# Simon-Kotchou/ViT.rs

Measured on AMD Instinct MI355X. Metric: images/sec (train step) ViT-B/16 224² bf16 at 1/2/4/8 MI355X; % MFMA roofline, higher is better.
Workload: dtype bf16; 1 GPU; vit_b16 224x224 train step (fwd+bwd+SGD), batch 256/GPU, bf16; model=vit_b16, global_batch=256, seq_len=197, parallelism=dp1

## Files before the change

### vit.rs_amd/csrc/gemm.h

```cpp
#pragma once
#include "common.h"

namespace vit {

enum Epi {
    EPI_F32_STORE = 0,
    EPI_F32_ACC = 1,
    EPI_F32_ATOMIC = 2,
    EPI_BF16_STORE = 3,
    EPI_BF16_GELU = 4,
    EPI_F32_RESID = 5,
    EPI_BF16_DGELU = 6,
    EPI_F32_SLAB = 7,
    EPI_BF16_GELU_D = 8,
    EPI_BF16_MUL = 9,
};
constexpr bool epi_aux16(int e) { return e == EPI_BF16_DGELU || e == EPI_BF16_MUL; }
constexpr bool epi_bias(int e) { return e != EPI_F32_ATOMIC && e != EPI_F32_SLAB && !epi_aux16(e); }
constexpr bool epi_mx(int e) { return e == EPI_BF16_GELU || e == EPI_BF16_GELU_D || epi_aux16(e); }

struct GemmArgs {
    const void* A = nullptr;
    long long lda = 0;
    bool a_kcontig = true;
    const void* B = nullptr;
    long long ldb = 0;
    bool b_kcontig = true;
    void* C = nullptr;
    long long ldc = 0;
    void* C2 = nullptr;
    const void* aux = nullptr;
    long long ldaux = 0;
    const float* bias = nullptr;
    float* dbias = nullptr;
    float* colsum_out = nullptr;
    float* colsum_part = nullptr;
    int M = 0, N = 0, K = 0;
    int epi = EPI_F32_STORE;
    int splitk = 0;
    int fill_pct = 0;
    float* ws = nullptr;
    size_t ws_bytes = 0;
    const void* a_scale = nullptr;
    const void* b_scale = nullptr;
    uint8_t* mx_q = nullptr;
    uint8_t* mx_s = nullptr;
    uint8_t* mxc_q = nullptr;
    uint8_t* mxc_s = nullptr;
    long long mxc_ld = 0;
    long long mxc_off = 0;
};

void gemm_f32(const GemmArgs& a, hipStream_t s);
void gemm_bf16(const GemmArgs& a, hipStream_t s);
bool gemm_bf16_supported(const GemmArgs& a);
void gemm_set_variant(int v);
void gemm_set_debug(int flags);
int gemm_cu_count();
int gemm_persist_grid();
struct GemmParams;
void gemm_set_trace(unsigned long long* trace);
bool gemm_pp_shape(const GemmArgs& a);
void gemm_bf16_pp(const GemmArgs& a, const GemmParams& p, hipStream_t s);
// ... 48 lines not shown
```

### vit.rs_amd/csrc/gemm.hip

```cpp
#include "gemm_common.h"

#include <cstdlib>

#ifndef VIT_G2_ONEPHASE
#define VIT_G2_ONEPHASE 0
#endif

namespace vit {

namespace bf {
constexpr int BM = 128, BN = 128, BK = 64, NT = 256;
constexpr int SK = 72;
constexpr int SMN = 144;
constexpr int TILE = 9216;
static_assert(BM * SK == TILE && BK * SMN == TILE, "image sizes");

template <bool KC, int ROWS>
struct Stager {
    uint4 r[4];
    __device__ __forceinline__ void load(const bf16_t* __restrict__ base, long long ld, int row0,
                                         int rows_lim, int k0, int k_lim, int tid) {
#pragma unroll
        for (int c = 0; c < 4; c++) {
            const int idx = c * NT + tid;
// ... 1187 lines not shown
    if (slab) slab_reduce(a, slab, split, s);
    if (a.dbias) colsum_bf16(a.dbias, (const bf16_t*)a.A, a.K, a.M, a.lda, s);
}

void gemm_bf16(const GemmArgs& a, hipStream_t s) {
    if (a.M <= 0 || a.N <= 0) return;
    if (a.mx_q || a.mxc_q) {
        set_error("gemm_bf16: the fused MX output is an fp8-engine feature");
        return;
    }
    if (!gemm_bf16_supported(a)) {
        set_error("gemm_bf16: unsupported shape/alignment M=%d N=%d K=%d lda=%lld ldb=%lld",
                  a.M, a.N, a.K, a.lda, a.ldb);
        return;
    }
    if (gemm_variant() != 1 && a.epi == EPI_F32_ATOMIC && !a.a_kcontig && !a.b_kcontig &&
        a.K % g4::KTILE == 0 && a.M >= 256 && a.N >= 128 && a.N % 4 == 0 &&
        (a.splitk > 0 || !a.ws ||
         (size_t)choose_split_g4(cdiv(a.M, g4::BM) * cdiv(a.N, g4::BN), a.K / g4::KTILE) * a.M * a.N * sizeof(float) <=
             a.ws_bytes)) {
        gemm_bf16_g4(a, s);
        return;
    }
    const bool big = a.K % g2::KTILE == 0 && a.M >= 256 && a.N >= 256 && gemm_variant() != 1;
    if (big) {
        const int tiles = cdiv(a.M, g2::BM) * cdiv(a.N, g2::BN);
        int split = 1;
        if (a.epi == EPI_F32_ATOMIC) split = a.splitk > 0 ? a.splitk : choose_split_waves(tiles, a.K / g2::KTILE);
        int kchunk = cdiv(cdiv(a.K, split), g2::KTILE) * g2::KTILE;
        split = cdiv(a.K, kchunk);
        GemmArgs b = a;
        float* slab = nullptr;
        if (a.epi == EPI_F32_ATOMIC) {
            if (split > 1) {
                if (!(slab = slab_buffer(a, split))) return;
                b.epi = EPI_F32_SLAB;
                b.C = slab;
                b.ldc = a.N;
            } else {
                b.epi = EPI_F32_ACC;
            }
        }
        GemmParams p = make_gemm_params(b, kchunk);
        p.tiles = tiles;
        float* cs_rows = colsum_rows_begin(a);
        if ((a.colsum_out || a.colsum_part) && epi_aux16(a.epi) && !cs_rows) return;
        p.colsum_out = cs_rows;
// ... 69 lines not shown
```

### vit.rs_amd/csrc/ops.hip

```cpp
#include "ops_internal.h"
#include "ln_common.h"

namespace vit {

__global__ void residual_fwd_k(float* __restrict__ out, const float* __restrict__ a,
                               const float* __restrict__ b, long long n) {
    for (long long i = blockIdx.x * (long long)blockDim.x + threadIdx.x; i < n;
         i += (long long)gridDim.x * blockDim.x)
        out[i] = a[i] + b[i];
}
__global__ void residual_bwd_k(float* __restrict__ d1, float* __restrict__ d2,
                               const float* __restrict__ dout, long long n) {
    for (long long i = blockIdx.x * (long long)blockDim.x + threadIdx.x; i < n;
         i += (long long)gridDim.x * blockDim.x) {
        const float g = dout[i];
        d1[i] += g;
        d2[i] += g;
    }
}
__global__ void gelu_fwd_k(float* __restrict__ out, const float* __restrict__ inp, long long n) {
    for (long long i = blockIdx.x * (long long)blockDim.x + threadIdx.x; i < n;
         i += (long long)gridDim.x * blockDim.x)
        out[i] = gelu_f(inp[i]);
}
// ... 101 lines not shown
    }
}
__global__ void f2bf_k(bf16_t* __restrict__ out, const float* __restrict__ inp, long long n) {
    for (long long i = blockIdx.x * (long long)blockDim.x + threadIdx.x; i < n;
         i += (long long)gridDim.x * blockDim.x)
        out[i] = f2bf(inp[i]);
}
__global__ void bf2f_k(float* __restrict__ out, const bf16_t* __restrict__ inp, long long n) {
    for (long long i = blockIdx.x * (long long)blockDim.x + threadIdx.x; i < n;
         i += (long long)gridDim.x * blockDim.x)
        out[i] = bf2f(inp[i]);
}

int grid_for(long long n, int threads) {
    long long b = (n + threads - 1) / threads;
    return (int)(b < 1 ? 1 : (b > 8192 ? 8192 : b));
}

template <typename TO>
__global__ __launch_bounds__(256) void ln_fwd_k(TO* __restrict__ out, float* __restrict__ mean,
                                                float* __restrict__ rstd,
                                                const float* __restrict__ inp,
                                                const float* __restrict__ w,
                                                const float* __restrict__ b, long long rows, int C) {
    const int lane = threadIdx.x & 63;
    const long long row = blockIdx.x * 4LL + (threadIdx.x >> 6);
    if (row >= rows) return;
    const float* x = inp + row * C;
    float s = 0.f;
    for (int i = lane; i < C; i += 64) s += x[i];
    const float m = warp_sum(s) / (float)C;
    float v = 0.f;
    for (int i = lane; i < C; i += 64) {
        const float d = x[i] - m;
        v += d * d;
    }
    v = warp_sum(v) / (float)C;
    const float r = 1.0f / sqrtf(v + 1e-5f);
    TO* o = out + row * C;
    for (int i = lane; i < C; i += 64) {
        const float y = (r * (x[i] - m)) * w[i] + b[i];
        if constexpr (sizeof(TO) == 2)
            o[i] = f2bf(y);
        else
            o[i] = y;
    }
    if (lane == 0) {
        mean[row] = m;
        rstd[row] = r;
    }
// ... 55 lines not shown
            dval -= nrm * dnorm_norm_mean;
            dval *= rs;
            const long long o = row * C + i;
            if constexpr (ST) {
                const float t = lo8_decode(bf2f(io.hi_in[o]), io.lo_in[o]) + dval;
                const bf16_t h = f2bf(t);
                io.hi_out[o] = h;
                io.lo_out[o] = (uint8_t)lo8_encode(t, bf2f(h));
                ps[i] += t;
            } else {
                io.dinp[o] += dval;
            }
        }
    }
    lnb_flush(io, sm, C);
}

template <int NV, typename TO>
__global__ __launch_bounds__(256) void ln_fwd_vec_k(TO* __restrict__ out, float* __restrict__ mean,
                                                    float* __restrict__ rstd,
                                                    const float* __restrict__ inp,
                                                    const float* __restrict__ w,
                                                    const float* __restrict__ b, long long rows,
                                                    int C) {
    const int lane = threadIdx.x & 63;
    const long long row = blockIdx.x * 4LL + (threadIdx.x >> 6);
    if (row >= rows) return;
    const float4* x4 = reinterpret_cast<const float4*>(inp + row * C);
    float4 v[NV];
#pragma unroll
    for (int j = 0; j < NV; j++) v[j] = x4[lane + 64 * j];
    float m, r;
    ln_vec_stats<NV>(v, C, m, r);
#pragma unroll
    for (int j = 0; j < NV; j++) {
        const int k = lane + 64 * j;
        const float4 y = ln_vec_y(v[j], reinterpret_cast<const float4*>(w)[k], reinterpret_cast<const float4*>(b)[k], m, r);
        if constexpr (sizeof(TO) == 2)
            reinterpret_cast<uint2*>(out + row * C)[k] = make_uint2(pack_bf16x2(y.x, y.y), pack_bf16x2(y.z, y.w));
        else
            reinterpret_cast<float4*>(out + row * C)[k] = y;
    }
    if (lane == 0) {
        mean[row] = m;
        rstd[row] = r;
    }
}

__device__ __forceinline__ float4 ld4(const float* p, int k) { return reinterpret_cast<const float4*>(p)[k]; }
__device__ __forceinline__ float4 ld4(const bf16_t* p, int k) {
// ... 403 lines not shown
    float s = 0.f;
    for (int y = 0; y < nch; y++) s += part[y * n + i];
    dwpe[i] += s;
    tsum[i] = s;
}
__global__ void patch_small_grads_fin_k(float* __restrict__ dcls, float* __restrict__ dpb,
                                        const float* __restrict__ tsum, int T, int C) {
    const int c = blockIdx.x * blockDim.x + threadIdx.x;
    if (c >= C) return;
    float ps[8] = {0.f, 0.f, 0.f, 0.f, 0.f, 0.f, 0.f, 0.f};
    int t = 1;
    for (; t + 8 <= T; t += 8) {
#pragma unroll
        for (int j = 0; j < 8; j++) ps[j] += tsum[(long long)(t + j) * C + c];
    }
    for (int j = 0; t < T; t++, j++) ps[j] += tsum[(long long)t * C + c];
    const float s = ((ps[0] + ps[1]) + (ps[2] + ps[3])) + ((ps[4] + ps[5]) + (ps[6] + ps[7]));
    dcls[c] += tsum[c];
    dpb[c] += s;
}

template <typename TO>
static void ln_forward_any(TO* out, float* mean, float* rstd, const float* inp, const float* w,
                           const float* b, long long rows, int C, hipStream_t s) {
    if (rows <= 0) return;
    const int g = cdiv(rows, 4);
    const bool vec = C % 256 == 0 && C <= 2048 && (((uintptr_t)inp | (uintptr_t)out | (uintptr_t)w | (uintptr_t)b) & 15) == 0;
    switch (vec ? C / 256 : 0) {
        case 1: ln_fwd_vec_k<1, TO><<<g, 256, 0, s>>>(out, mean, rstd, inp, w, b, rows, C); break;
        case 2: ln_fwd_vec_k<2, TO><<<g, 256, 0, s>>>(out, mean, rstd, inp, w, b, rows, C); break;
        case 3: ln_fwd_vec_k<3, TO><<<g, 256, 0, s>>>(out, mean, rstd, inp, w, b, rows, C); break;
        case 4: ln_fwd_vec_k<4, TO><<<g, 256, 0, s>>>(out, mean, rstd, inp, w, b, rows, C); break;
        case 5: ln_fwd_vec_k<5, TO><<<g, 256, 0, s>>>(out, mean, rstd, inp, w, b, rows, C); break;
        case 6: ln_fwd_vec_k<6, TO><<<g, 256, 0, s>>>(out, mean, rstd, inp, w, b, rows, C); break;
        case 8: ln_fwd_vec_k<8, TO><<<g, 256, 0, s>>>(out, mean, rstd, inp, w, b, rows, C); break;
        default: ln_fwd_k<TO><<<g, 256, 0, s>>>(out, mean, rstd, inp, w, b, rows, C); break;
    }
    after_launch("layernorm_forward");
}
void ln_forward_f32(float* out, float* mean, float* rstd, const float* inp, const float* w,
                    const float* b, long long rows, int C, hipStream_t s) {
    ln_forward_any<float>(out, mean, rstd, inp, w, b, rows, C, s);
}
void ln_forward_bf16(bf16_t* out, float* mean, float* rstd, const float* inp, const float* w,
                     const float* b, long long rows, int C, hipStream_t s) {
    ln_forward_any<bf16_t>(out, mean, rstd, inp, w, b, rows, C, s);
}
int ln_bwd_blocks(long long rows);
template <typename TD, bool ST>
static void ln_backward_any(LnbIo io, const TD* dout, const float* inp, const float* w,
                            const float* mean, const float* rstd, long long rows, int C, hipStream_t s,
                            float* ws = nullptr) {
    if (rows <= 0) return;
    const bool reduce = io.part == nullptr;
    const int nsum = io.dsum ? 3 * C : 2 * C;
    if (reduce) {
        io.part = ws ? ws : (float*)workspace((size_t)ln_bwd_blocks(rows) * nsum * sizeof(float));
        if (!io.part) return;
    }
    const bool vec = C % 256 == 0 && C <= 2048 &&
                     (((uintptr_t)io.dinp | (uintptr_t)dout | (uintptr_t)inp | (uintptr_t)w |
                       (uintptr_t)io.hi_in | (uintptr_t)io.hi_out | (uintptr_t)io.lo_in | (uintptr_t)io.lo_out) & 15) == 0;
    const int grid = ln_bwd_blocks(rows);
    const size_t lds = 12 * (size_t)C * sizeof(float);
    if (lds > 160 * 1024) { set_error("layernorm_backward: C=%d exceeds the LDS column partials", C); return; }
    if (!vec) {
        if (lds > 64 * 1024) VIT_HIP(hipFuncSetAttribute((const void*)ln_bwd_k<TD, ST>,
                                                         hipFuncAttributeMaxDynamicSharedMemorySize, (int)lds));
        ln_bwd_k<TD, ST><<<grid, 256, lds, s>>>(io, dout, inp, w, mean, rstd, rows, C);
// ... 499 lines not shown
```

### vit.rs_amd/csrc/ops_internal.h

```cpp
#pragma once
#include "common.h"
#include "gemm.h"
#include "../../include/vit_ops.h"

namespace vit {
int grid_for(long long n, int threads);
void ln_forward_f32(float* out, float* mean, float* rstd, const float* inp, const float* w,
                    const float* b, long long rows, int C, hipStream_t s);
void ln_forward_bf16(bf16_t* out, float* mean, float* rstd, const float* inp, const float* w,
                     const float* b, long long rows, int C, hipStream_t s);
void ln_backward_f32(float* dinp, float* dw, float* db, const float* dout, const float* inp,
                     const float* w, const float* mean, const float* rstd, long long rows, int C,
                     hipStream_t s, float* ws = nullptr);
void ln_backward_bf16_stream(bf16_t* dres_out, uint8_t* lo_out, const bf16_t* dres_in, const uint8_t* lo_in,
                             float* dw, float* db, float* dres_colsum, const bf16_t* dout, const float* inp,
                             const float* w, const float* mean, const float* rstd, long long rows, int C,
                             hipStream_t s, float* part = nullptr);
int ln_bwd_blocks(long long rows);
void convert_f2bf(bf16_t* out, const float* inp, long long n, hipStream_t s);
void sgd(float* p, const float* g, long long n, float lr, hipStream_t s);
void sgd_clip(float* p, const float* g, long long n, float lr, const ClipRec* rec, hipStream_t s);
int group_grid(int ntiles);
void sgd_groups(float* p, const float* g, const GroupTab& gt, int tile_begin, int ntiles, float lr,
                const ClipRec* rec, hipStream_t s);
int sumsq_blocks(long long n);
void sumsq_partials(double* slots, const float* x, long long n, hipStream_t s);
void sumsq_finish(double* out, const double* slots, int nslots, hipStream_t s);
void clip_finish(ClipRec* rec, const double* slots, int nslots, float max_norm, hipStream_t s);
void softmax_rows(float* probs, const float* logits, long long rows, int V, hipStream_t s);
void ce_forward(float* losses, const float* probs, const int* targets, long long rows, int V,
                hipStream_t s);
void ce_backward(float* dlogits, const float* dlosses, const float* probs, const int* targets,
                 long long rows, int V, hipStream_t s);
// ... 38 lines not shown
```

### vit.rs_amd/csrc/trainer.hip

```cpp
#include <rccl/rccl.h>

#include <algorithm>
#include <cmath>
#include <cstdlib>
#include <cstring>
#include <string>
#include <vector>

#include "ops_internal.h"
#include "../../include/vit_trainer.h"
#include "../../include/vit_checkpoint.h"
#include "../../include/vit_data.h"
#include "../../include/vit_jpeg.h"

namespace vit {
bool jpeg_loader_decode_to(vit_jpeg_loader_t* l, uint8_t* out, int img, hipStream_t st, const int** labels,
                           int expect_n);
namespace {

enum TIdx {
    P_PATCH_W, P_PATCH_B, P_CLS, P_WPE, P_LN1W, P_LN1B, P_QKVW, P_QKVB, P_ATTPROJW, P_ATTPROJB,
    P_LN2W, P_LN2B, P_FCW, P_FCB, P_FCPROJW, P_FCPROJB, P_LNFW, P_LNFB, P_HEADW, P_HEADB
};

// ... 239 lines not shown
}

struct DevBuf {
    void* p = nullptr;
    size_t bytes = 0;
};

}

struct Trainer {
    vit_config_t cfg{};
    int B = 0, T = 0, NP = 0, C = 0, L = 0, NH = 0, NC = 0, KP = 0, prec = 0, device = 0;
    long long BT = 0;
    long long n_params = 0;
    long long arena_elems = 0;
    long long canon_size[20]{};
    std::vector<long long> off;
    long long chunk_off[VIT_MAX_LAYERS + 3]{};
    int n_chunks = 0;

    hipStream_t s = nullptr, s_comm = nullptr;
    hipStream_t s2 = nullptr;
    bool two_streams = true;
    enum BwdEv { EV_RESA, EV_RESB, EV_DFCH, EV_DQKV, EV_W1, EV_W2, EV_W3, EV_W4, EV_JOIN, EV_SG, EV_PRE_IN, EV_PRE, EV_COUNT };
    hipEvent_t bev[EV_COUNT]{};
    static constexpr int MAXMB = 4;
    int nmb = 1, mb_want = 2;
    int pick_nmb(int want) const {
        if (!two_streams) return 1;
        for (int k = want < MAXMB ? want : MAXMB; k >= 2; k--)
            if (B % k == 0) return k;
        return 1;
    }
    hipStream_t ms[MAXMB]{};
    hipEvent_t mev[MAXMB][EV_COUNT]{};
    hipEvent_t fork_ev = nullptr, join_ev[MAXMB]{};
    std::vector<hipEvent_t> chunk_evm;
    std::vector<hipEvent_t> chunk_ev2;
    std::vector<hipEvent_t> chunk_ev;
    hipEvent_t comm_done = nullptr;

    float* params = nullptr;
    float* grads = nullptr;
    float* gemm_ws = nullptr;
    float* attn_part = nullptr;
    size_t gemm_ws_bytes = 0;
    bf16_t* pbf = nullptr;
// ... 341 lines not shown
            } else {
                patches_bf = alloc<bf16_t>((long long)B * NP * KPP);
            }
            if (patch_pad) {
                wpatch_pad = alloc<bf16_t>((long long)C * KPP);
                dwpatch_pad = alloc<float>((long long)C * KPP);
                if (wpatch_pad) VIT_HIP(hipMemset(wpatch_pad, 0, (size_t)C * KPP * 2));
            }
            for (int l = 0; l < L; l++) {
                LayerActs& a = la[l];
                a.ln1 = alloc<bf16_t>(BT * C);
                a.ln1_mean = alloc<float>(BT);
                a.ln1_rstd = alloc<float>(BT);
                a.qkv = alloc<bf16_t>(BT * 3 * C);
                a.atty = alloc<bf16_t>(BT * C);
                a.lse = alloc<float>(BT * NH);
                a.res2 = alloc<float>(BT * C);
                a.ln2 = alloc<bf16_t>(BT * C);
                a.ln2_mean = alloc<float>(BT);
                a.ln2_rstd = alloc<float>(BT);
                a.fchd = alloc<bf16_t>(BT * 4 * C);
                a.fchg = alloc<bf16_t>(BT * 4 * C);
                a.res3 = alloc<float>(BT * C);
            }
            dln_bf = alloc<bf16_t>(BT * C);
            dres_bf = alloc<bf16_t>(BT * C);
            dres_bf2 = alloc<bf16_t>(BT * C);
            dres_lo = alloc<uint8_t>(BT * C);
            dres_lo2 = alloc<uint8_t>(BT * C);
            dfch = alloc<bf16_t>(BT * 4 * C);
            datty = alloc<bf16_t>(BT * C);
            dqkv = alloc<bf16_t>(BT * 3 * C);
            if (!patch_f32) dpatch_bf = alloc<bf16_t>((long long)B * NP * C);
            gemm_ws_bytes = (size_t)32 * 4 * C * (size_t)std::max(C, KP) * sizeof(float);
            gemm_ws = alloc<float>((long long)(gemm_ws_bytes / sizeof(float)));
            attn_part = alloc<float>((long long)attn_backward_ws_floats(B, T, C, NH) + MAXMB * 3LL * C);
            {
                const long long lnr = (long long)MAXMB * ln_bwd_blocks(BT), fcr = cdiv(BT, 96) + MAXMB;
                sg_ln2 = 0;
                sg_ln1 = sg_ln2 + lnr * 3 * C;
                sg_fcb = sg_ln1 + lnr * 3 * C;
                sg_qkv = sg_fcb + fcr * 4 * C;
                const long long n = sg_qkv + (long long)MAXMB * 3 * C;
                sg_part[0] = alloc<float>(n);
                sg_part[1] = alloc<float>(n);
            }
// ... 201 lines not shown
            aq = act_q2[mb];
            as = act_s2[mb];
        } else if (pre == PRE_NONE) {
            tbeg(TC_QUANT, 0, st);
            if (colq) {
                const long long r0 = (long long)mb * (B / nmb) * T;
                const long long ntok = mb_ntok(mb, a.M);
                quantize_mx_rowcol_bf16(act_q[mb], act_s[mb], colq->q, colq->s, (const bf16_t*)a.A, a.M, a.K, a.lda,
                                        kp_tok, r0, ntok, st);
            } else {
                quantize_mx_bf16(act_q[mb], act_s[mb], (const bf16_t*)a.A, a.M, a.K, a.lda, a.K, st);
            }
            tend();
            if (rec_ev >= 0 && two_streams) VIT_HIP(hipEventRecord(mev[mb][rec_ev], st));
        }
        const QMat w = transposed ? wtq_of(ti, l) : wq_of(ti, l);
        a.A = aq; a.lda = a.K; a.a_scale = as;
        a.B = w.q; a.ldb = a.K; a.b_scale = w.s; a.b_kcontig = true;
        tbeg(cls, 2.0 * a.M * (double)a.N * a.K, st);
        gemm_fp8(a, st);
        tend();
    }

    bool head_sk = true;
    bool patch_tail = true;
    int head_split(int M, int N, int K) const {
        if (!head_sk) return 0;
        int sp = std::min(16, std::max(1, K / 64));
        while (sp > 1 && (size_t)sp * M * N * sizeof(float) > gemm_ws_bytes) sp--;
        return sp;
    }
    void head_forward() {
        tbeg(TC_HEAD, 2.0 * B * C * NC);
        const float* last = la[L - 1].res3;
        VIT_HIP(hipMemcpy2DAsync(cls_x, C * 4, last, (size_t)T * C * 4, C * 4, B, hipMemcpyDeviceToDevice, s));
        ln_forward_f32(lnf, lnf_mean, lnf_rstd, cls_x, P(P_LNFW), P(P_LNFB), B, C, s);
        GemmArgs a;
        a.A = lnf; a.lda = C; a.B = P(P_HEADW); a.ldb = C; a.C = logits; a.ldc = NC;
        a.bias = P(P_HEADB); a.M = B; a.N = NC; a.K = C; a.epi = EPI_F32_STORE;
        if (lowp()) {
            bcast_rows_k<<<cdiv((long long)B * NC, 256), 256, 0, s>>>(logits, P(P_HEADB), B, NC);
            a.bias = nullptr;
            a.epi = EPI_F32_ATOMIC;
            a.splitk = head_split(a.M, a.N, a.K);
        }
        a.ws = gemm_ws; a.ws_bytes = gemm_ws_bytes;
// ... 28 lines not shown
        w.A = dlogits; w.lda = NC; w.a_kcontig = false;
        w.B = lnf; w.ldb = C; w.b_kcontig = false;
        w.C = G(P_HEADW); w.ldc = C; w.M = NC; w.N = C; w.K = B; w.epi = lowp() ? EPI_F32_ATOMIC : EPI_F32_ACC;
        if (lowp()) w.splitk = head_split(w.M, w.N, w.K);
        w.ws = gemm_ws; w.ws_bytes = gemm_ws_bytes;
        gemm_f32(w, s);
        colsum_f32(G(P_HEADB), dlogits, B, NC, NC, s, red_ws);
        VIT_HIP(hipMemsetAsync(dcls_x, 0, (size_t)B * C * 4, s));
        ln_backward_f32(dcls_x, G(P_LNFW), G(P_LNFB), dlnf, cls_x, P(P_LNFW), lnf_mean, lnf_rstd, B, C, s, red_ws);
        if (dres_bf) {
            VIT_HIP(hipMemsetAsync(dres_bf, 0, (size_t)BT * C * 2, s));
            VIT_HIP(hipMemsetAsync(dres_lo, 0, (size_t)BT * C, s));
            rows_to_bf16_k<<<cdiv((long long)B * C, 256), 256, 0, s>>>(dres_bf, dres_lo, (long long)T * C, dcls_x, B, C);
        } else {
            VIT_HIP(hipMemsetAsync(dres, 0, (size_t)BT * C * 4, s));
            VIT_HIP(hipMemcpy2DAsync(dres, (size_t)T * C * 4, dcls_x, C * 4, C * 4, B, hipMemcpyDeviceToDevice, s));
        }
        tend();
    }

    void forward_bf16() {
        const int Bm = B / nmb;
        const long long R = (long long)Bm * T;
        mb_fork();
        for (int mb = 0; mb < nmb; mb++) {
            hipStream_t st = ms[mb];
            const long long img0 = (long long)mb * Bm;
            tbeg(TC_PATCH, 2.0 * Bm * NP * (double)KP * C, st);
            GemmArgs a;
            a.C = emb_tmp + img0 * NP * C; a.ldc = C; a.bias = P(P_PATCH_B);
            a.M = Bm * NP; a.N = C; a.K = KP; a.epi = EPI_F32_STORE;
            if (patch_f32) {
                im2col_f32(patches_f + img0 * NP * KP, pixels + img0 * 3 * cfg.img * cfg.img, Bm, cfg.img,
                           cfg.patch, st);
                a.A = patches_f + img0 * NP * KP; a.lda = KP; a.B = P(P_PATCH_W); a.ldb = KP;
                gemm_f32(a, st);
            } else if (patch_pad) {
                im2col_pad_bf16(patches_bf + img0 * NP * KPP, pixels + img0 * 3 * cfg.img * cfg.img, Bm, cfg.img,
                                cfg.patch, KPP, st);
                a.A = patches_bf + img0 * NP * KPP; a.lda = KPP; a.B = wpatch_pad; a.ldb = KPP; a.K = KPP;
                gemm_bf16(a, st);
            } else {
                im2col_bf16(patches_bf + img0 * NP * KP, pixels + img0 * 3 * cfg.img * cfg.img, Bm, cfg.img,
                            cfg.patch, st);
                a.A = patches_bf + img0 * NP * KP; a.lda = KP; a.B = W(P_PATCH_W); a.ldb = KP;
                gemm_bf16(a, st);
            }
            patch_assemble(encoded + img0 * T * C, emb_tmp + img0 * NP * C, P(P_CLS), P(P_WPE), Bm, NP, C, st);
            tend();
        }
        for (int l = 0; l < L; l++) {
            LayerActs& a = la[l];
            const float* xl = l == 0 ? encoded : la[l - 1].res3;
            for (int mb = 0; mb < nmb; mb++) {
                hipStream_t st = ms[mb];
                const long long r0 = (long long)mb * R;
                const float* x = xl + r0 * C;
                const bool rc = rowcol_on(), lm = lnmx_on();
                QMat c_ln1 = rc ? actc_of(0, l) : QMat{}, c_atty = rc ? actc_of(1, l) : QMat{},
                     c_ln2 = rc ? actc_of(2, l) : QMat{};
                tbeg(TC_LN_FWD, 0, st);
                if (lm)
                    ln_forward_mx(act_q[mb], act_s[mb], c_ln1.q, c_ln1.s, a.ln1_mean + r0, a.ln1_rstd + r0, x,
                                  P(P_LN1W, l), P(P_LN1B, l), R, C, kp_tok, r0, mb_ntok(mb, R), st,
                                  ln_left ? lnb_scr[mb] : nullptr);
                else
                    ln_forward_bf16(a.ln1 + r0 * C, a.ln1_mean + r0, a.ln1_rstd + r0, x, P(P_LN1W, l), P(P_LN1B, l), R, C, st);
                tend();
                GemmArgs q;
                q.A = a.ln1 + r0 * C; q.lda = C; q.B = W(P_QKVW, l); q.ldb = C; q.C = a.qkv + r0 * 3 * C;
                q.ldc = 3 * C; q.bias = P(P_QKVB, l); q.M = (int)R; q.N = 3 * C; q.K = C; q.epi = EPI_BF16_STORE;
                gemm_w(TC_QKV_FWD, q, P_QKVW, l, false, mb, st, lm ? PRE_LN : PRE_NONE, false,
                       rc && !lm ? &c_ln1 : nullptr);
                tbeg(TC_ATTN_FWD, 4.0 * Bm * (double)T * T * C, st);
                attn_forward_fused(a.atty + r0 * C, a.lse + (long long)mb * Bm * NH * T, a.qkv + r0 * 3 * C, Bm, T, C, NH, st);
                tend();
                GemmArgs pr;
                pr.A = a.atty + r0 * C; pr.lda = C; pr.B = W(P_ATTPROJW, l); pr.ldb = C; pr.C = a.res2 + r0 * C;
                pr.ldc = C; pr.bias = P(P_ATTPROJB, l); pr.aux = x; pr.ldaux = C;
                pr.M = (int)R; pr.N = C; pr.K = C; pr.epi = EPI_F32_RESID;
                gemm_w(TC_PROJ_FWD, pr, P_ATTPROJW, l, false, mb, st, PRE_NONE, false, rc ? &c_atty : nullptr);
                tbeg(TC_LN_FWD, 0, st);
                if (lm)
                    ln_forward_mx(act_q[mb], act_s[mb], c_ln2.q, c_ln2.s, a.ln2_mean + r0, a.ln2_rstd + r0,
                                  a.res2 + r0 * C, P(P_LN2W, l), P(P_LN2B, l), R, C, kp_tok, r0, mb_ntok(mb, R), st,
                                  ln_left ? lnb_scr[mb] : nullptr);
                else
                    ln_forward_bf16(a.ln2 + r0 * C, a.ln2_mean + r0, a.ln2_rstd + r0, a.res2 + r0 * C, P(P_LN2W, l),
                                    P(P_LN2B, l), R, C, st);
                tend();
                GemmArgs f;
                f.A = a.ln2 + r0 * C; f.lda = C; f.B = W(P_FCW, l); f.ldb = C; f.C = a.fchd + r0 * 4 * C;
                f.C2 = a.fchg + r0 * 4 * C; f.ldc = 4 * C; f.bias = P(P_FCB, l); f.M = (int)R; f.N = 4 * C;
                f.K = C; f.epi = EPI_BF16_GELU_D;
                if (epicol_on()) {
                    const QMat g = fchgc_of(l);
                    f.C2 = nullptr;
                    f.mxc_q = g.q; f.mxc_s = g.s; f.mxc_ld = kp_tok; f.mxc_off = r0;
                }
                gemm_w(TC_FC_FWD, f, P_FCW, l, false, mb, st, lm ? PRE_LN : PRE_NONE, fuse_mx,
                       rc && !lm ? &c_ln2 : nullptr);
                GemmArgs fp;
                fp.A = a.fchg + r0 * 4 * C; fp.lda = 4 * C; fp.B = W(P_FCPROJW, l); fp.ldb = 4 * C;
                fp.C = a.res3 + r0 * C; fp.ldc = C; fp.bias = P(P_FCPROJB, l); fp.aux = a.res2 + r0 * C;
                fp.ldaux = C; fp.M = (int)R; fp.N = C; fp.K = 4 * C; fp.epi = EPI_F32_RESID;
                gemm_w(TC_FCPROJ_FWD, fp, P_FCPROJW, l, false, mb, st, fuse_mx ? PRE_EPI : PRE_NONE);
            }
        }
        mb_join();
        head_forward();
    }

    void wgrad(int cls, const bf16_t* dout, int OC, const bf16_t* inp, int Cin, float* dW, int ready,
               int done, const QMat* dout_c = nullptr, const QMat* inp_c = nullptr) {
        GemmArgs w;
        w.A = dout; w.lda = OC; w.a_kcontig = false;
        w.B = inp; w.ldb = Cin; w.b_kcontig = false;
        w.C = dW; w.ldc = Cin; w.M = OC; w.N = Cin; w.K = (int)BT; w.epi = EPI_F32_ATOMIC;
        w.ws = gemm_ws; w.ws_bytes = gemm_ws_bytes;
        w.fill_pct = two_streams ? 0 : 80;
        hipStream_t st = two_streams ? s2 : s;
        if (two_streams) {
            for (int mb = 0; mb < nmb; mb++) {
                if (!dout_c) VIT_HIP(hipEventRecord(mev[mb][ready], ms[mb]));
                VIT_HIP(hipStreamWaitEvent(s2, mev[mb][ready], 0));
            }
        }
        if (fp8() && fp8_wgrad) {
// ... 31 lines not shown
                VIT_HIP(hipStreamWaitEvent(s2, mev[mb][EV_SG], 0));
            }
        }
        const int nb = nmb * ln_bwd_blocks(R), w1 = l > 0 ? 3 * C : 2 * C;
        const float* p2 = sg_rows(l, sg_ln2);
        const float* p1 = sg_rows(l, sg_ln1);
        RowsJob jobs[8] = {
            {G(P_LN2W, l), p2, nb, 3 * C, C},
            {G(P_LN2B, l), p2 + C, nb, 3 * C, C},
            {G(P_ATTPROJB, l), p2 + 2 * C, nb, 3 * C, C},
            {G(P_LN1W, l), p1, nb, w1, C},
            {G(P_LN1B, l), p1 + C, nb, w1, C},
            {G(P_FCB, l), sg_rows(l, sg_fcb), nmb * fcb_rows, 4 * C, 4 * C},
            {G(P_QKVB, l), sg_rows(l, sg_qkv), nmb, 3 * C, 3 * C},
            {l > 0 ? G(P_FCPROJB, l - 1) : nullptr, p1 + 2 * C, nb, w1, C},
        };
        tbeg(TC_COLSUM, 0, st);
        rows_reduce_add(jobs, l > 0 ? 8 : 7, st);
        tend();
    }

    void backward_bf16() {
        pre_side_wait();
        bf16_t* rbA = dres_bf;
        bf16_t* rbB = dres_bf2;
        uint8_t* loA = dres_lo;
        uint8_t* loB = dres_lo2;
        head_backward(nullptr, rbA, loA);
        chunk_done(0);
        colsum_f32(G(P_FCPROJB, L - 1), dcls_x, B, C, C, s, red_ws);
        mb_fork();
        const int Bm = B / nmb;
        const long long R = (long long)Bm * T;
        for (int l = L - 1; l >= 0; l--) {
            LayerActs& a = la[l];
            const float* xl = l == 0 ? encoded : la[l - 1].res3;
            const bool rc = rowcol_on();
            QMat c_ln1 = rc ? actc_of(0, l) : QMat{}, c_atty = rc ? actc_of(1, l) : QMat{}, c_ln2 = rc ? actc_of(2, l) : QMat{};
            const bool lbm = lnbmx_on(), resa_pre = lbm && l < L - 1;
            const bool ec = epicol_on();
            QMat c_fchg = ec ? fchgc_of(l) : QMat{};
            if (!rc) wgrad(TC_FCPROJ_WGRAD, rbA, C, a.fchg, 4 * C, G(P_FCPROJW, l), EV_RESA, EV_W1);
            for (int mb = 0; mb < nmb; mb++) {
                const long long r0 = mb * R;
                after_wgrad(EV_W2, ms[mb]);
                GemmArgs d1;
                d1.A = rbA + r0 * C; d1.lda = C; dgrad_b(d1, P_FCPROJW, l, C, 4 * C);
                d1.C = dfch + r0 * 4 * C; d1.ldc = 4 * C; d1.aux = a.fchd + r0 * 4 * C; d1.ldaux = 4 * C;
                d1.M = (int)R; d1.N = 4 * C; d1.K = C; d1.epi = EPI_BF16_MUL;
                fcb_rows = gemm_colsum_rows(d1, fp8());
                d1.colsum_part = sg_rows(l, sg_fcb) + (long long)mb * fcb_rows * 4 * C;
                if (ec) {
                    d1.C = nullptr;
                    d1.mxc_q = dfchc.q; d1.mxc_s = dfchc.s; d1.mxc_ld = kp_tok; d1.mxc_off = r0;
                }
                gemm_w(TC_FCPROJ_DGRAD, d1, P_FCPROJW, l, true, mb, ms[mb], resa_pre ? PRE_LN : PRE_NONE, fuse_mx,
                       rc && !resa_pre ? &dcol[0] : nullptr, resa_pre ? -1 : EV_RESA);
                if (ec && two_streams) VIT_HIP(hipEventRecord(mev[mb][EV_DFCH], ms[mb]));
            }
            if (rc) wgrad(TC_FCPROJ_WGRAD, rbA, C, a.fchg, 4 * C, G(P_FCPROJW, l), EV_RESA, EV_W1, &dcol[0],
                          ec ? &c_fchg : nullptr);
            wgrad(TC_FC_WGRAD, dfch, 4 * C, a.ln2, C, G(P_FCW, l), EV_DFCH, EV_W2, ec ? &dfchc : nullptr,
                  rc ? &c_ln2 : nullptr);
            for (int mb = 0; mb < nmb; mb++) {
                const long long r0 = mb * R;
                GemmArgs d2;
                d2.A = dfch + r0 * 4 * C; d2.lda = 4 * C; dgrad_b(d2, P_FCW, l, 4 * C, C);
                d2.C = dln_bf + r0 * C; d2.ldc = C; d2.M = (int)R; d2.N = C; d2.K = 4 * C; d2.epi = EPI_BF16_STORE;
                gemm_w(TC_FC_DGRAD, d2, P_FCW, l, true, mb, ms[mb], fuse_mx ? PRE_EPI : PRE_NONE);
                after_wgrad(EV_W3, ms[mb]);
                tbeg(TC_LN_BWD, 0, ms[mb]);
                if (lbm) {
                    ln_backward_bf16_stream_mx(rbB + r0 * C, loB + r0 * C, rbA + r0 * C, loA + r0 * C, G(P_LN2W, l),
                                               G(P_LN2B, l), G(P_ATTPROJB, l), dln_bf + r0 * C, a.res2 + r0 * C,
                                               P(P_LN2W, l), a.ln2_mean + r0, a.ln2_rstd + r0, R, C, ms[mb],
                                               sg_rows(l, sg_ln2) + (long long)mb * ln_bwd_blocks(R) * 3 * C,
                                               act_q[mb], act_s[mb], dcol[1].q, dcol[1].s, kp_tok, r0, mb_ntok(mb, R),
                                               lnb_scr[mb]);
                    if (two_streams) VIT_HIP(hipEventRecord(mev[mb][EV_RESB], ms[mb]));
                } else {
                    ln_backward_bf16_stream(rbB + r0 * C, loB + r0 * C, rbA + r0 * C, loA + r0 * C, G(P_LN2W, l),
                                            G(P_LN2B, l), G(P_ATTPROJB, l), dln_bf + r0 * C, a.res2 + r0 * C,
                                            P(P_LN2W, l), a.ln2_mean + r0, a.ln2_rstd + r0, R, C, ms[mb],
                                            sg_rows(l, sg_ln2) + (long long)mb * ln_bwd_blocks(R) * 3 * C);
                }
                tend();
            }
            if (!rc) wgrad(TC_PROJ_WGRAD, rbB, C, a.atty, C, G(P_ATTPROJW, l), EV_RESB, EV_W3);
            for (int mb = 0; mb < nmb; mb++) {
                const long long r0 = mb * R;
                GemmArgs d3;
                d3.A = rbB + r0 * C; d3.lda = C; dgrad_b(d3, P_ATTPROJW, l, C, C);
                d3.C = datty + r0 * C; d3.ldc = C; d3.M = (int)R; d3.N = C; d3.K = C; d3.epi = EPI_BF16_STORE;
                gemm_w(TC_PROJ_DGRAD, d3, P_ATTPROJW, l, true, mb, ms[mb], lbm ? PRE_LN : PRE_NONE, false,
                       rc && !lbm ? &dcol[1] : nullptr, lbm ? -1 : EV_RESB);
                after_wgrad(EV_W4, ms[mb]);
                tbeg(TC_ATTN_BWD, 8.0 * Bm * (double)T * T * C, ms[mb]);
                attn_backward_fused(dqkv + r0 * 3 * C, datty + r0 * C, a.qkv + r0 * 3 * C, a.atty + r0 * C,
                                    a.lse + (long long)mb * Bm * NH * T, Bm, T, C, NH, ms[mb],
                                    sg_rows(l, sg_qkv) + (long long)mb * 3 * C,
                                    attn_part + (long long)attn_backward_ws_floats(mb * Bm, T, C, NH), true);
                tend();
            }
            if (rc) wgrad(TC_PROJ_WGRAD, rbB, C, a.atty, C, G(P_ATTPROJW, l), EV_RESB, EV_W3, &dcol[1], &c_atty);
            if (!rc) wgrad(TC_QKV_WGRAD, dqkv, 3 * C, a.ln1, C, G(P_QKVW, l), EV_DQKV, EV_W4);
            for (int mb = 0; mb < nmb; mb++) {
                const long long r0 = mb * R;
                GemmArgs d4;
                d4.A = dqkv + r0 * 3 * C; d4.lda = 3 * C; dgrad_b(d4, P_QKVW, l, 3 * C, C);
                d4.C = dln_bf + r0 * C; d4.ldc = C; d4.M = (int)R; d4.N = C; d4.K = 3 * C; d4.epi = EPI_BF16_STORE;
                gemm_w(TC_QKV_DGRAD, d4, P_QKVW, l, true, mb, ms[mb], PRE_NONE, false, rc ? &dcol[2] : nullptr, EV_DQKV);
                after_wgrad(EV_W1, ms[mb]);
                tbeg(TC_LN_BWD, 0, ms[mb]);
                if (lbm && l > 0) {
                    ln_backward_bf16_stream_mx(rbA + r0 * C, loA + r0 * C, rbB + r0 * C, loB + r0 * C, G(P_LN1W, l),
                                               G(P_LN1B, l), G(P_FCPROJB, l - 1), dln_bf + r0 * C, xl + r0 * C,
// ... 933 lines not shown
    const std::string n = name ? name : "";
    if (n == "microbatch") {
        t.mb_want = value;
        t.nmb = t.pick_nmb(value);
    } else if (n == "dgrad_transposed") {
        t.dgrad_wt = value != 0;
    } else if (n == "fp8_ln_mx") {
        t.ln_mx = value != 0;
    } else if (n == "fp8_ln_leftover") {
        t.ln_left = value != 0;
    } else if (n == "early_sgd") {
        t.early_sgd = value < 0 ? -1 : value != 0;
    } else if (n == "pre_side") {
        t.pre_side_wait();
        t.pre_side = value != 0;
    } else if (n == "patch_tail") {
        t.patch_tail = value != 0;
    } else if (n == "head_splitk") {
        t.head_sk = value != 0;
    } else if (n == "fp8_lnb_mx") {
        t.lnb_mx = value != 0;
    } else if (n == "clip_overlap") {
        t.clip_overlap = value < 0 ? -1 : value != 0;
    } else if (n == "dp_probe") {
        if (value && !t.dp_snap) {
            t.dp_snap = t.alloc<float>(t.arena_elems);
            if (t.dp_snap) VIT_HIP(hipMemset(t.dp_snap, 0, t.arena_elems * 4));
        }
        t.dp_probe_on = value != 0 && t.dp_snap != nullptr;
    } else {
        set_error("vit_trainer_set_option: unknown option '%s'", n.c_str());
        return 1;
    }
    return vit::has_error();
}
int vit_trainer_set_timing(vit_trainer_t* h, int on) {
    h->t.timing = on != 0;
    return 0;
}
int vit_trainer_timing(vit_trainer_t* h, const char** names, double* ms, long long* calls,
                       double* flops, int max) {
    auto& t = h->t;
    t.collect();
    int n = 0;
    for (int c = 0; c < vit::TC_COUNT && n < max; c++) {
        if (!t.t_calls[c]) continue;
// ... 19 lines not shown
```

Before: 7226 images/s.

## Compute only CLS-token rows in the last transformer block after attention

In the final layer, the attention projection, LN2, MLP forward GEMMs and the corresponding backward dgrads run only on the CLS row of each image. This uses a row stride of T, so M becomes the batch size instead of batch×197. The change targets the wasted MLP and projection FLOPs on tokens whose outputs never reach the classifier head. Non-CLS outputs are zero-initialised, and the dgrad output buffers are re-memset each step on a side stream. This adds complexity and relies on the head consuming only the CLS token, which is mathematically exact for ViT classification. The wgrad paths still use full buffers, which are zero on the skipped rows.

```diff
diff --git a/vit.rs_amd/csrc/gemm.h b/vit.rs_amd/csrc/gemm.h
--- a/vit.rs_amd/csrc/gemm.h
+++ b/vit.rs_amd/csrc/gemm.h
@@ -39,6 +39,7 @@
     int epi = EPI_F32_STORE;
     int splitk = 0;
     int fill_pct = 0;
+    bool rows_gathered = false;
     float* ws = nullptr;
     size_t ws_bytes = 0;
     const void* a_scale = nullptr;
diff --git a/vit.rs_amd/csrc/gemm.hip b/vit.rs_amd/csrc/gemm.hip
--- a/vit.rs_amd/csrc/gemm.hip
+++ b/vit.rs_amd/csrc/gemm.hip
@@ -1233,7 +1233,8 @@
         gemm_bf16_g4(a, s);
         return;
     }
-    const bool big = a.K % g2::KTILE == 0 && a.M >= 256 && a.N >= 256 && gemm_variant() != 1;
+    const bool gathered = a.rows_gathered && a.M >= 1 && a.a_kcontig && a.epi != EPI_F32_ATOMIC;
+    const bool big = a.K % g2::KTILE == 0 && (a.M >= 256 || gathered) && a.N >= 256 && gemm_variant() != 1;
     if (big) {
         const int tiles = cdiv(a.M, g2::BM) * cdiv(a.N, g2::BN);
         int split = 1;
diff --git a/vit.rs_amd/csrc/ops.hip b/vit.rs_amd/csrc/ops.hip
--- a/vit.rs_amd/csrc/ops.hip
+++ b/vit.rs_amd/csrc/ops.hip
@@ -147,10 +147,11 @@
                                                 float* __restrict__ rstd,
                                                 const float* __restrict__ inp,
                                                 const float* __restrict__ w,
-                                                const float* __restrict__ b, long long rows, int C) {
+                                                const float* __restrict__ b, long long rows, int C,
+                                                long long rstride) {
     const int lane = threadIdx.x & 63;
-    const long long row = blockIdx.x * 4LL + (threadIdx.x >> 6);
-    if (row >= rows) return;
+    if (blockIdx.x * 4LL + (threadIdx.x >> 6) >= rows) return;
+    const long long row = (blockIdx.x * 4LL + (threadIdx.x >> 6)) * rstride;
     const float* x = inp + row * C;
     float s = 0.f;
     for (int i = lane; i < C; i += 64) s += x[i];
@@ -252,10 +253,10 @@
                                                     const float* __restrict__ inp,
                                                     const float* __restrict__ w,
                                                     const float* __restrict__ b, long long rows,
-                                                    int C) {
+                                                    int C, long long rstride) {
     const int lane = threadIdx.x & 63;
-    const long long row = blockIdx.x * 4LL + (threadIdx.x >> 6);
-    if (row >= rows) return;
+    if (blockIdx.x * 4LL + (threadIdx.x >> 6) >= rows) return;
+    const long long row = (blockIdx.x * 4LL + (threadIdx.x >> 6)) * rstride;
     const float4* x4 = reinterpret_cast<const float4*>(inp + row * C);
     float4 v[NV];
 #pragma unroll
@@ -705,19 +706,19 @@
 
 template <typename TO>
 static void ln_forward_any(TO* out, float* mean, float* rstd, const float* inp, const float* w,
-                           const float* b, long long rows, int C, hipStream_t s) {
+                           const float* b, long long rows, int C, hipStream_t s, long long rstride = 1) {
     if (rows <= 0) return;
     const int g = cdiv(rows, 4);
     const bool vec = C % 256 == 0 && C <= 2048 && (((uintptr_t)inp | (uintptr_t)out | (uintptr_t)w | (uintptr_t)b) & 15) == 0;
     switch (vec ? C / 256 : 0) {
-        case 1: ln_fwd_vec_k<1, TO><<<g, 256, 0, s>>>(out, mean, rstd, inp, w, b, rows, C); break;
-        case 2: ln_fwd_vec_k<2, TO><<<g, 256, 0, s>>>(out, mean, rstd, inp, w, b, rows, C); break;
-        case 3: ln_fwd_vec_k<3, TO><<<g, 256, 0, s>>>(out, mean, rstd, inp, w, b, rows, C); break;
-        case 4: ln_fwd_vec_k<4, TO><<<g, 256, 0, s>>>(out, mean, rstd, inp, w, b, rows, C); break;
-        case 5: ln_fwd_vec_k<5, TO><<<g, 256, 0, s>>>(out, mean, rstd, inp, w, b, rows, C); break;
-        case 6: ln_fwd_vec_k<6, TO><<<g, 256, 0, s>>>(out, mean, rstd, inp, w, b, rows, C); break;
-        case 8: ln_fwd_vec_k<8, TO><<<g, 256, 0, s>>>(out, mean, rstd, inp, w, b, rows, C); break;
-        default: ln_fwd_k<TO><<<g, 256, 0, s>>>(out, mean, rstd, inp, w, b, rows, C); break;
+        case 1: ln_fwd_vec_k<1, TO><<<g, 256, 0, s>>>(out, mean, rstd, inp, w, b, rows, C, rstride); break;
+        case 2: ln_fwd_vec_k<2, TO><<<g, 256, 0, s>>>(out, mean, rstd, inp, w, b, rows, C, rstride); break;
+        case 3: ln_fwd_vec_k<3, TO><<<g, 256, 0, s>>>(out, mean, rstd, inp, w, b, rows, C, rstride); break;
+        case 4: ln_fwd_vec_k<4, TO><<<g, 256, 0, s>>>(out, mean, rstd, inp, w, b, rows, C, rstride); break;
+        case 5: ln_fwd_vec_k<5, TO><<<g, 256, 0, s>>>(out, mean, rstd, inp, w, b, rows, C, rstride); break;
+        case 6: ln_fwd_vec_k<6, TO><<<g, 256, 0, s>>>(out, mean, rstd, inp, w, b, rows, C, rstride); break;
+        case 8: ln_fwd_vec_k<8, TO><<<g, 256, 0, s>>>(out, mean, rstd, inp, w, b, rows, C, rstride); break;
+        default: ln_fwd_k<TO><<<g, 256, 0, s>>>(out, mean, rstd, inp, w, b, rows, C, rstride); break;
     }
     after_launch("layernorm_forward");
 }
@@ -726,8 +727,8 @@
     ln_forward_any<float>(out, mean, rstd, inp, w, b, rows, C, s);
 }
 void ln_forward_bf16(bf16_t* out, float* mean, float* rstd, const float* inp, const float* w,
-                     const float* b, long long rows, int C, hipStream_t s) {
-    ln_forward_any<bf16_t>(out, mean, rstd, inp, w, b, rows, C, s);
+                     const float* b, long long rows, int C, hipStream_t s, long long row_stride) {
+    ln_forward_any<bf16_t>(out, mean, rstd, inp, w, b, rows, C, s, row_stride);
 }
 int ln_bwd_blocks(long long rows);
 template <typename TD, bool ST>
diff --git a/vit.rs_amd/csrc/ops_internal.h b/vit.rs_amd/csrc/ops_internal.h
--- a/vit.rs_amd/csrc/ops_internal.h
+++ b/vit.rs_amd/csrc/ops_internal.h
@@ -8,7 +8,7 @@
 void ln_forward_f32(float* out, float* mean, float* rstd, const float* inp, const float* w,
                     const float* b, long long rows, int C, hipStream_t s);
 void ln_forward_bf16(bf16_t* out, float* mean, float* rstd, const float* inp, const float* w,
-                     const float* b, long long rows, int C, hipStream_t s);
+                     const float* b, long long rows, int C, hipStream_t s, long long row_stride = 1);
 void ln_backward_f32(float* dinp, float* dw, float* db, const float* dout, const float* inp,
                      const float* w, const float* mean, const float* rstd, long long rows, int C,
                      hipStream_t s, float* ws = nullptr);
diff --git a/vit.rs_amd/csrc/trainer.hip b/vit.rs_amd/csrc/trainer.hip
--- a/vit.rs_amd/csrc/trainer.hip
+++ b/vit.rs_amd/csrc/trainer.hip
@@ -285,7 +285,7 @@
     hipStream_t s = nullptr, s_comm = nullptr;
     hipStream_t s2 = nullptr;
     bool two_streams = true;
-    enum BwdEv { EV_RESA, EV_RESB, EV_DFCH, EV_DQKV, EV_W1, EV_W2, EV_W3, EV_W4, EV_JOIN, EV_SG, EV_PRE_IN, EV_PRE, EV_COUNT };
+    enum BwdEv { EV_RESA, EV_RESB, EV_DFCH, EV_DQKV, EV_W1, EV_W2, EV_W3, EV_W4, EV_JOIN, EV_SG, EV_PRE_IN, EV_PRE, EV_LC_IN, EV_LC, EV_COUNT };
     hipEvent_t bev[EV_COUNT]{};
     static constexpr int MAXMB = 4;
     int nmb = 1, mb_want = 2;
@@ -673,6 +673,15 @@
                 a.fchd = alloc<bf16_t>(BT * 4 * C);
                 a.fchg = alloc<bf16_t>(BT * 4 * C);
                 a.res3 = alloc<float>(BT * C);
+            }
+            if (prec == VIT_BF16 && !has_error()) {
+                LayerActs& a = la[L - 1];
+                VIT_HIP(hipMemsetAsync(a.ln2_mean, 0, (size_t)BT * 4, s));
+                VIT_HIP(hipMemsetAsync(a.ln2_rstd, 0, (size_t)BT * 4, s));
+                VIT_HIP(hipMemsetAsync(a.res2, 0, (size_t)BT * C * 4, s));
+                VIT_HIP(hipMemsetAsync(a.ln2, 0, (size_t)BT * C * 2, s));
+                VIT_HIP(hipMemsetAsync(a.fchd, 0, (size_t)BT * 4 * C * 2, s));
+                VIT_HIP(hipMemsetAsync(a.fchg, 0, (size_t)BT * 4 * C * 2, s));
             }
             dln_bf = alloc<bf16_t>(BT * C);
             dres_bf = alloc<bf16_t>(BT * C);
@@ -920,6 +929,33 @@
         tend();
     }
 
+    bool last_cls = true;
+    bool lc_active = false;
+    bool lc_dirty = true;
+    bool lc_pending = false;
+    bool last_cls_on() const { return last_cls && prec == VIT_BF16; }
+    void last_cls_clear() {
+        if (!lc_dirty) return;
+        hipStream_t cs = s;
+        if (two_streams && s2) {
+            VIT_HIP(hipEventRecord(bev[EV_LC_IN], s));
+            VIT_HIP(hipStreamWaitEvent(s2, bev[EV_LC_IN], 0));
+            cs = s2;
+        }
+        VIT_HIP(hipMemsetAsync(dln_bf, 0, (size_t)BT * C * 2, cs));
+        VIT_HIP(hipMemsetAsync(datty, 0, (size_t)BT * C * 2, cs));
+        if (cs != s) {
+            VIT_HIP(hipEventRecord(bev[EV_LC], cs));
+            lc_pending = true;
+        }
+        lc_dirty = false;
+    }
+    void last_cls_wait() {
+        if (!lc_pending) return;
+        VIT_HIP(hipStreamWaitEvent(s, bev[EV_LC], 0));
+        lc_pending = false;
+    }
+
     bool head_sk = true;
     bool patch_tail = true;
     int head_split(int M, int N, int K) const {
@@ -994,6 +1030,8 @@
     void forward_bf16() {
         const int Bm = B / nmb;
         const long long R = (long long)Bm * T;
+        lc_active = last_cls_on();
+        if (lc_active) last_cls_clear();
         mb_fork();
         for (int mb = 0; mb < nmb; mb++) {
             hipStream_t st = ms[mb];
@@ -1024,6 +1062,10 @@
         for (int l = 0; l < L; l++) {
             LayerActs& a = la[l];
             const float* xl = l == 0 ? encoded : la[l - 1].res3;
+            const bool lc = lc_active && l == L - 1;
+            const int Mr = lc ? Bm : (int)R;
+            const long long rs = lc ? T : 1;
+            const bool lcg = lc && R >= 256;
             for (int mb = 0; mb < nmb; mb++) {
                 hipStream_t st = ms[mb];
                 const long long r0 = (long long)mb * R;
@@ -1048,9 +1090,9 @@
                 attn_forward_fused(a.atty + r0 * C, a.lse + (long long)mb * Bm * NH * T, a.qkv + r0 * 3 * C, Bm, T, C, NH, st);
                 tend();
                 GemmArgs pr;
-                pr.A = a.atty + r0 * C; pr.lda = C; pr.B = W(P_ATTPROJW, l); pr.ldb = C; pr.C = a.res2 + r0 * C;
-                pr.ldc = C; pr.bias = P(P_ATTPROJB, l); pr.aux = x; pr.ldaux = C;
-                pr.M = (int)R; pr.N = C; pr.K = C; pr.epi = EPI_F32_RESID;
+                pr.A = a.atty + r0 * C; pr.lda = rs * C; pr.B = W(P_ATTPROJW, l); pr.ldb = C; pr.C = a.res2 + r0 * C;
+                pr.ldc = rs * C; pr.bias = P(P_ATTPROJB, l); pr.aux = x; pr.ldaux = rs * C;
+                pr.M = Mr; pr.N = C; pr.K = C; pr.epi = EPI_F32_RESID; pr.rows_gathered = lcg;
                 gemm_w(TC_PROJ_FWD, pr, P_ATTPROJW, l, false, mb, st, PRE_NONE, false, rc ? &c_atty : nullptr);
                 tbeg(TC_LN_FWD, 0, st);
                 if (lm)
@@ -1059,12 +1101,12 @@
                                   ln_left ? lnb_scr[mb] : nullptr);
                 else
                     ln_forward_bf16(a.ln2 + r0 * C, a.ln2_mean + r0, a.ln2_rstd + r0, a.res2 + r0 * C, P(P_LN2W, l),
-                                    P(P_LN2B, l), R, C, st);
+                                    P(P_LN2B, l), Mr, C, st, rs);
                 tend();
                 GemmArgs f;
-                f.A = a.ln2 + r0 * C; f.lda = C; f.B = W(P_FCW, l); f.ldb = C; f.C = a.fchd + r0 * 4 * C;
-                f.C2 = a.fchg + r0 * 4 * C; f.ldc = 4 * C; f.bias = P(P_FCB, l); f.M = (int)R; f.N = 4 * C;
-                f.K = C; f.epi = EPI_BF16_GELU_D;
+                f.A = a.ln2 + r0 * C; f.lda = rs * C; f.B = W(P_FCW, l); f.ldb = C; f.C = a.fchd + r0 * 4 * C;
+                f.C2 = a.fchg + r0 * 4 * C; f.ldc = rs * 4 * C; f.bias = P(P_FCB, l); f.M = Mr; f.N = 4 * C;
+                f.K = C; f.epi = EPI_BF16_GELU_D; f.rows_gathered = lcg;
                 if (epicol_on()) {
                     const QMat g = fchgc_of(l);
                     f.C2 = nullptr;
@@ -1073,9 +1115,9 @@
                 gemm_w(TC_FC_FWD, f, P_FCW, l, false, mb, st, lm ? PRE_LN : PRE_NONE, fuse_mx,
                        rc && !lm ? &c_ln2 : nullptr);
                 GemmArgs fp;
-                fp.A = a.fchg + r0 * 4 * C; fp.lda = 4 * C; fp.B = W(P_FCPROJW, l); fp.ldb = 4 * C;
-                fp.C = a.res3 + r0 * C; fp.ldc = C; fp.bias = P(P_FCPROJB, l); fp.aux = a.res2 + r0 * C;
-                fp.ldaux = C; fp.M = (int)R; fp.N = C; fp.K = 4 * C; fp.epi = EPI_F32_RESID;
+                fp.A = a.fchg + r0 * 4 * C; fp.lda = rs * 4 * C; fp.B = W(P_FCPROJW, l); fp.ldb = 4 * C;
+                fp.C = a.res3 + r0 * C; fp.ldc = rs * C; fp.bias = P(P_FCPROJB, l); fp.aux = a.res2 + r0 * C;
+                fp.ldaux = rs * C; fp.M = Mr; fp.N = C; fp.K = 4 * C; fp.epi = EPI_F32_RESID; fp.rows_gathered = lcg;
                 gemm_w(TC_FCPROJ_FWD, fp, P_FCPROJW, l, false, mb, st, fuse_mx ? PRE_EPI : PRE_NONE);
             }
         }
@@ -1153,6 +1195,8 @@
 
     void backward_bf16() {
         pre_side_wait();
+        last_cls_wait();
+        lc_dirty = true;
         bf16_t* rbA = dres_bf;
         bf16_t* rbB = dres_bf2;
         uint8_t* loA = dres_lo;
@@ -1166,6 +1210,10 @@
         for (int l = L - 1; l >= 0; l--) {
             LayerActs& a = la[l];
             const float* xl = l == 0 ? encoded : la[l - 1].res3;
+            const bool lc = lc_active && l == L - 1;
+            const int Mr = lc ? Bm : (int)R;
+            const long long rs = lc ? T : 1;
+            const bool lcg = lc && R >= 256;
             const bool rc = rowcol_on();
             QMat c_ln1 = rc ? actc_of(0, l) : QMat{}, c_atty = rc ? actc_of(1, l) : QMat{}, c_ln2 = rc ? actc_of(2, l) : QMat{};
             const bool lbm = lnbmx_on(), resa_pre = lbm && l < L - 1;
@@ -1196,8 +1244,9 @@
             for (int mb = 0; mb < nmb; mb++) {
                 const long long r0 = mb * R;
                 GemmArgs d2;
-                d2.A = dfch + r0 * 4 * C; d2.lda = 4 * C; dgrad_b(d2, P_FCW, l, 4 * C, C);
-                d2.C = dln_bf + r0 * C; d2.ldc = C; d2.M = (int)R; d2.N = C; d2.K = 4 * C; d2.epi = EPI_BF16_STORE;
+                d2.A = dfch + r0 * 4 * C; d2.lda = rs * 4 * C; dgrad_b(d2, P_FCW, l, 4 * C, C);
+                d2.C = dln_bf + r0 * C; d2.ldc = rs * C; d2.M = Mr; d2.N = C; d2.K = 4 * C; d2.epi = EPI_BF16_STORE;
+                d2.rows_gathered = lcg;
                 gemm_w(TC_FC_DGRAD, d2, P_FCW, l, true, mb, ms[mb], fuse_mx ? PRE_EPI : PRE_NONE);
                 after_wgrad(EV_W3, ms[mb]);
                 tbeg(TC_LN_BWD, 0, ms[mb]);
@@ -1221,8 +1270,9 @@
             for (int mb = 0; mb < nmb; mb++) {
                 const long long r0 = mb * R;
                 GemmArgs d3;
-                d3.A = rbB + r0 * C; d3.lda = C; dgrad_b(d3, P_ATTPROJW, l, C, C);
-                d3.C = datty + r0 * C; d3.ldc = C; d3.M = (int)R; d3.N = C; d3.K = C; d3.epi = EPI_BF16_STORE;
+                d3.A = rbB + r0 * C; d3.lda = rs * C; dgrad_b(d3, P_ATTPROJW, l, C, C);
+                d3.C = datty + r0 * C; d3.ldc = rs * C; d3.M = Mr; d3.N = C; d3.K = C; d3.epi = EPI_BF16_STORE;
+                d3.rows_gathered = lcg;
                 gemm_w(TC_PROJ_DGRAD, d3, P_ATTPROJW, l, true, mb, ms[mb], lbm ? PRE_LN : PRE_NONE, false,
                        rc && !lbm ? &dcol[1] : nullptr, lbm ? -1 : EV_RESB);
                 after_wgrad(EV_W4, ms[mb]);
@@ -2202,6 +2252,8 @@
         t.lnb_mx = value != 0;
     } else if (n == "clip_overlap") {
         t.clip_overlap = value < 0 ? -1 : value != 0;
+    } else if (n == "last_cls") {
+        t.last_cls = value != 0;
     } else if (n == "dp_probe") {
         if (value && !t.dp_snap) {
             t.dp_snap = t.alloc<float>(t.arena_elems);
```

New measurement: 7372 images/s, median of 6. +2.0%, better.
